# ZeayW/Multimodal-fusion-based-Pre-routing-Timing-Prediction-

Measured on AMD Instinct MI355X. Metric: train-step samples/sec, higher is better.
Workload: dtype bf16; 1 GPU; config B: 8 designs/step/GPU, 65536-node netlist, 64 levels, 256x256 tile, 1350 endpoints/design, UNet(max), bf16 operands / fp32 accumulate on the MFMA-bound contractions; U-Net activations and their gradients stored bf16, netlist tensors, statistics, parameters and gradients fp32; nodes=65536, levels=64, tile=256, endpoints_per_design=1350, cone_pruning=False, parallelism=dp1 (designs sharded, one all-reduce of the flat gradient per step), launch=one HIP graph replay per step (Adam inside)

## Files before the change

multimodal-fusion-based-pre-routing-timing-prediction-_amd/csrc/mlp_feat.hip:

```cpp
#include <stdlib.h>
#include "mlp_tile_bf16.h"
#include "mlp_feat_frag.h"
#include "tr_read.h"
#include "../../include/mmft_incr.h"

namespace mmft {

int launch_slab_reduce(const float* slabs, int splits, long long elems, float* out, int accumulate, hipStream_t st);

struct FeatFwdArgs {
  const float* x;
  long long ldx;
  int row0, n, fin;
  const float *w1, *b1, *w2, *b2;
  float* out;
  long long ldout;
  int relu_out;
  const unsigned char* active;
};

template <int KS, bool MASKED>
__global__ void __launch_bounds__(512) mlp2_feat_fwd_kernel(FeatFwdArgs a) {
  constexpr int BM = 64, RT = BM / 16, XS = KS * 32 + 8, HS = L2_HD + 8;
  __shared__ __attribute__((aligned(16))) unsigned short xs[BM * XS];
  __shared__ __attribute__((aligned(16))) unsigned short hs[BM * HS];
  const int tid = threadIdx.x, lane = tid & 63, wave = tid >> 6;
  const int r16 = lane & 15, q = lane >> 4;
  const int ntiles = (a.n + BM - 1) / BM;
  auto next_tile = [&](int t, unsigned long long& flags) -> int {
    if constexpr (MASKED) {
      for (; t < ntiles; t += (int)gridDim.x) {
        const int m = t * BM + lane;
        flags = __ballot(m < a.n && a.active[a.row0 + m] != 0);
        if (flags) break;
      }
    }
    return t;
  };
  unsigned long long flags = ~0ull;
  int tile = next_tile(blockIdx.x, flags);
  if constexpr (MASKED) {
    if (tile >= ntiles) return;
  }
  bf16x8 w1f[2][KS], w2f[8];
#pragma unroll
  for (int j = 0; j < 2; ++j)
#pragma unroll
    for (int ks = 0; ks < KS; ++ks) w1f[j][ks] = mf_w1_frag(a.w1, a.fin, wave * 32 + j * 16 + r16, ks * 32 + q * 8);
#pragma unroll
  for (int ks = 0; ks < 8; ++ks) w2f[ks] = mf_pack8(a.w2 + (long long)(wave * 16 + r16) * L2_HD + ks * 32 + q * 8);
  const int nn2 = wave * 16 + q * 4;
  const f32x4 b2v = *reinterpret_cast<const f32x4*>(a.b2 + nn2);
  f32x4 b1v[2];
#pragma unroll
  for (int j = 0; j < 2; ++j) b1v[j] = *reinterpret_cast<const f32x4*>(a.b1 + wave * 32 + j * 16 + q * 4);
  constexpr int NXE = BM * KS * 32 / 512;
  float xr[NXE];
  auto request = [&](int tile) {
#pragma unroll
    for (int k = 0; k < NXE; ++k) {
      const int e = tid + k * 512, r = e / (KS * 32), kk = e % (KS * 32);
      const int m = tile * BM + r;
      xr[k] = (m < a.n && kk < a.fin) ? a.x[(long long)(a.row0 + m) * a.ldx + kk] : 0.f;
    }
  };
  if (tile < ntiles) request(tile);
  while (tile < ntiles) {
    const int m0 = tile * BM;
#pragma unroll
    for (int k = 0; k < NXE; ++k) {
      const int e = tid + k * 512;
      xs[(e / (KS * 32)) * XS + e % (KS * 32)] = mf_bf16(xr[k]);
    }
    __syncthreads();
    unsigned long long nflags = ~0ull;
    const int nxt = next_tile(tile + (int)gridDim.x, nflags);
    if (nxt < ntiles) request(nxt);
    f32x4 acc1[RT][2];
    tile_layer1<KS, RT>(acc1, w1f, xs, XS, r16, q);
#pragma unroll
    for (int i = 0; i < RT; ++i)
#pragma unroll
      for (int j = 0; j < 2; ++j) st_bf16x4(hs + (i * 16 + r16) * HS + wave * 32 + j * 16 + q * 4, relu4(acc1[i][j] + b1v[j]));
    __syncthreads();
    f32x4 acc2[RT];
#pragma unroll
    for (int i = 0; i < RT; ++i) acc2[i] = tile_layer2(w2f, hs, HS, r16, q, i);
#pragma unroll
    for (int i = 0; i < RT; ++i) {
      const int m = m0 + i * 16 + r16;
      if (m >= a.n) continue;
      if constexpr (MASKED) {
        if (!((flags >> (i * 16 + r16)) & 1)) continue;
      }
      f32x4 v = acc2[i] + b2v;
      if (a.relu_out) v = relu4(v);
      *reinterpret_cast<f32x4*>(a.out + (long long)(a.row0 + m) * a.ldout + nn2) = v;
    }
    __syncthreads();
    tile = nxt;
    flags = nflags;
  }
}

struct FeatBwdArgs {
  const float* g;
  long long ldg;
  const float* x;
  long long ldx;
  int row0, n, fin;
  const float *w1, *b1, *w2;
  float* slabs;
  long long slab;
};

template <int KS>
__global__ void __launch_bounds__(512) mlp2_feat_bwd_kernel(FeatBwdArgs a) {
  constexpr int BM = 32, KP = KS * 32, XS = KP + 16, GS = L2_D2 + 16, HS = L2_HD + 16, KB = KP / 16;
  extern __shared__ __attribute__((aligned(16))) unsigned short lds[];
  unsigned short* xs = lds;
  unsigned short* gs = xs + BM * XS;
  unsigned short* hs = gs + BM * GS;
  unsigned short* ds = hs + BM * HS;
  f32x4(*gred)[32] = reinterpret_cast<f32x4(*)[32]>(hs);
  const int tid = threadIdx.x, lane = tid & 63, wave = tid >> 6;
  const int r16 = lane & 15, q = lane >> 4;
  const int trr = tr_lane_row(lane), trc = tr_lane_col(lane);
  const f32x4 zero = {0.f, 0.f, 0.f, 0.f};

  bf16x8 w1f[2][KS], w2tf[2][4];
  f32x4 b1v[2];
#pragma unroll
  for (int j = 0; j < 2; ++j) {
    const int col = wave * 32 + j * 16 + r16;
#pragma unroll
    for (int ks = 0; ks < KS; ++ks) w1f[j][ks] = mf_w1_frag(a.w1, a.fin, col, ks * 32 + q * 8);
#pragma unroll
    for (int ks = 0; ks < 4; ++ks) {
      float v[8];
#pragma unroll
      for (int t = 0; t < 8; ++t) v[t] = a.w2[(long long)(ks * 32 + q * 8 + t) * L2_HD + col];
      w2tf[j][ks] = mf_pack8(v);
    }
    b1v[j] = *reinterpret_cast<const f32x4*>(a.b1 + wave * 32 + j * 16 + q * 4);
  }
  f32x4 dw2[2][8], dw1[2][KB], dsum[2], gsum = zero;
#pragma unroll
  for (int j = 0; j < 2; ++j) {
    dsum[j] = zero;
#pragma unroll
    for (int d = 0; d < 8; ++d) dw2[j][d] = zero;
#pragma unroll
    for (int k = 0; k < KB; ++k) dw1[j][k] = zero;
  }

  const int ntiles = (a.n + BM - 1) / BM;
  constexpr int NXE = BM * KP / 512;
  f32x4 gr[2];
  float xr[NXE];
  auto request = [&](int tile) {
    const int m0 = tile * BM;
#pragma unroll
    for (int it = 0; it < 2; ++it) {
      const int e = tid + it * 512, r = e >> 5, c = (e & 31) * 4;
      gr[it] = m0 + r < a.n ? *reinterpret_cast<const f32x4*>(a.g + (long long)(a.row0 + m0 + r) * a.ldg + c) : zero;
    }
#pragma unroll
    for (int k = 0; k < NXE; ++k) {
      const int e = tid + k * 512, r = e / KP, kk = e % KP;
      xr[k] = (m0 + r < a.n && kk < a.fin) ? a.x[(long long)(a.row0 + m0 + r) * a.ldx + kk] : 0.f;
    }
  };
  if ((int)blockIdx.x < ntiles) request(blockIdx.x);
  for (int tile = blockIdx.x; tile < ntiles; tile += gridDim.x) {
#pragma unroll
    for (int it = 0; it < 2; ++it) {
      const int e = tid + it * 512, r = e >> 5, c = (e & 31) * 4;
      const f32x4 v = gr[it];
      gsum += v;
      const unsigned lo = pack_bf16(v.x, v.y), hi = pack_bf16(v.z, v.w);
      *reinterpret_cast<unsigned long long*>(gs + r * GS + c) = ((unsigned long long)hi << 32) | lo;
    }
#pragma unroll
    for (int k = 0; k < NXE; ++k) {
      const int e = tid + k * 512, r = e / KP, kk = e % KP;
      xs[r * XS + kk] = mf_bf16(xr[k]);
    }
    __syncthreads();
    if (tile + (int)gridDim.x < ntiles) request(tile + gridDim.x);
    __syncthreads();
#pragma unroll
    for (int i = 0; i < 2; ++i) {
      f32x4 acc1[2] = {zero, zero}, acc3[2] = {zero, zero};
#pragma unroll
      for (int ks = 0; ks < KS; ++ks) {
        const bf16x8 xf = *reinterpret_cast<const bf16x8*>(xs + (i * 16 + r16) * XS + ks * 32 + q * 8);
#pragma unroll
        for (int j = 0; j < 2; ++j) acc1[j] = __builtin_amdgcn_mfma_f32_16x16x32_bf16(w1f[j][ks], xf, acc1[j], 0, 0, 0);
      }
#pragma unroll
      for (int ks = 0; ks < 4; ++ks) {
        const bf16x8 gf = *reinterpret_cast<const bf16x8*>(gs + (i * 16 + r16) * GS + ks * 32 + q * 8);
#pragma unroll
        for (int j = 0; j < 2; ++j) acc3[j] = __builtin_amdgcn_mfma_f32_16x16x32_bf16(w2tf[j][ks], gf, acc3[j], 0, 0, 0);
      }
      const int m = i * 16 + r16;
#pragma unroll
      for (int j = 0; j < 2; ++j) {
        const int nn = wave * 32 + j * 16 + q * 4;
        f32x4 hv = acc1[j] + b1v[j], dh = acc3[j];
#pragma unroll
        for (int t = 0; t < 4; ++t) {
          hv[t] = hv[t] > 0.f ? hv[t] : 0.f;
          dh[t] = hv[t] > 0.f ? dh[t] : 0.f;
        }
        dsum[j] += dh;
        const unsigned hl = pack_bf16(hv.x, hv.y), hh = pack_bf16(hv.z, hv.w);
        const unsigned dl = pack_bf16(dh.x, dh.y), dhh = pack_bf16(dh.z, dh.w);
        *reinterpret_cast<unsigned long long*>(hs + m * HS + nn) = ((unsigned long long)hh << 32) | hl;
        *reinterpret_cast<unsigned long long*>(ds + m * HS + nn) = ((unsigned long long)dhh << 32) | dl;
      }
    }
    __syncthreads();
#pragma unroll
    for (int j = 0; j < 2; ++j) {
      const int col0 = wave * 32 + j * 16;
      const bf16x8 hf = __builtin_bit_cast(bf16x8, tr_read_pair(hs + trr * HS + col0 + trc, 16 * HS));
      const bf16x8 df = __builtin_bit_cast(bf16x8, tr_read_pair(ds + trr * HS + col0 + trc, 16 * HS));
#pragma unroll
      for (int d = 0; d < 8; ++d) {
        const bf16x8 gf = __builtin_bit_cast(bf16x8, tr_read_pair(gs + trr * GS + d * 16 + trc, 16 * GS));
        dw2[j][d] = __builtin_amdgcn_mfma_f32_16x16x32_bf16(hf, gf, dw2[j][d], 0, 0, 0);
      }
#pragma unroll
      for (int k = 0; k < KB; ++k) {
        const bf16x8 xf = __builtin_bit_cast(bf16x8, tr_read_pair(xs + trr * XS + k * 16 + trc, 16 * XS));
        dw1[j][k] = __builtin_amdgcn_mfma_f32_16x16x32_bf16(df, xf, dw1[j][k], 0, 0, 0);
      }
    }
    __syncthreads();
  }

  float* sl = a.slabs + (long long)blockIdx.x * a.slab;
  float* s_dw1 = sl;
  float* s_db1 = s_dw1 + (long long)L2_HD * a.fin;
  float* s_dw2 = s_db1 + L2_HD;
  float* s_db2 = s_dw2 + (long long)L2_D2 * L2_HD;
#pragma unroll
  for (int j = 0; j < 2; ++j) {
    const int colq = wave * 32 + j * 16 + q * 4;
#pragma unroll
    for (int d = 0; d < 8; ++d) *reinterpret_cast<f32x4*>(s_dw2 + (long long)(d * 16 + r16) * L2_HD + colq) = dw2[j][d];
#pragma unroll
    for (int k = 0; k < KB; ++k) {
      const int kk = k * 16 + r16;
      if (kk < a.fin) {
#pragma unroll
        for (int t = 0; t < 4; ++t) s_dw1[(long long)(colq + t) * a.fin + kk] = dw1[j][k][t];
      }
    }
    f32x4 v = dsum[j];
#pragma unroll
    for (int o = 1; o < 16; o <<= 1) {
#pragma unroll
      for (int t = 0; t < 4; ++t) v[t] += __shfl_xor(v[t], o, 64);
    }
    if (r16 == 0) *reinterpret_cast<f32x4*>(s_db1 + colq) = v;
  }
  __syncthreads();
  gred[tid >> 5][tid & 31] = gsum;
  __syncthreads();
  if (tid < 32) {
    f32x4 v = gred[0][tid];
    for (int p = 1; p < 16; ++p) v += gred[p][tid];
    *reinterpret_cast<f32x4*>(s_db2 + tid * 4) = v;
  }
}

template <int KS>
constexpr int feat_bwd_lds() {
  constexpr int BM = 32, KP = KS * 32, XS = KP + 16, GS = L2_D2 + 16, HS = L2_HD + 16;
  return (BM * XS + BM * GS + 2 * BM * HS) * 2;
}

static inline long long feat_slab(int fin) { return (long long)L2_HD * fin + L2_HD + (long long)L2_D2 * L2_HD + L2_D2; }
static inline int feat_bwd_grid(int n) {
  int tiles = cdiv(n, 32);
  static int cap = getenv("MMFT_FEAT_BWD_GRID") ? atoi(getenv("MMFT_FEAT_BWD_GRID")) : 192;
  if (cap < 1) cap = 1;
  return tiles < cap ? (tiles < 1 ? 1 : tiles) : cap;
}

}

using namespace mmft;

static int feat_fwd_launch(const char* what, const float* x, long long ldx, int row0, int n, int fin, const float* w1,
                           const float* b1, const float* w2, const float* b2, float* out, long long ldout, int relu_out,
                           const unsigned char* active, int device, void* stream) {
  MMFT_REQUIRE(x && w1 && b1 && w2 && b2 && out, "%s: null pointer", what);
  MMFT_REQUIRE(n >= 0 && row0 >= 0 && fin >= 1 && fin <= 64 && ldx >= fin, "%s: bad sizes (fin <= 64)", what);
  MMFT_REQUIRE(ldout % 4 == 0 && aligned16(out) && aligned16(w2) && aligned16(b1) && aligned16(b2),
               "%s: out / w2 / biases must be 16-byte aligned", what);
  if (n == 0) return MMFT_OK;
  DeviceGuard dg(device);
  FeatFwdArgs a{x, ldx, row0, n, fin, w1, b1, w2, b2, out, ldout, relu_out, active};
  const double fl = 2.0 * n * ((double)fin * L2_HD + (double)L2_HD * L2_D2), by = 4.0 * n * ((double)fin + L2_D2);
  int grid = cdiv(n, 64);
  if (grid > 768) grid = 768;
  if (active) {
    if (fin <= 32)
      MMFT_LAUNCH("mlp2_feat_fwd_masked_kernel", fl, by, (mlp2_feat_fwd_kernel<1, true>), dim3(grid), dim3(512), (hipStream_t)stream, a);
    else
      MMFT_LAUNCH("mlp2_feat_fwd_masked_kernel", fl, by, (mlp2_feat_fwd_kernel<2, true>), dim3(grid), dim3(512), (hipStream_t)stream, a);
  } else if (fin <= 32)
    MMFT_LAUNCH("mlp2_feat_fwd_kernel", fl, by, (mlp2_feat_fwd_kernel<1, false>), dim3(grid), dim3(512), (hipStream_t)stream, a);
  else
    MMFT_LAUNCH("mlp2_feat_fwd_kernel", fl, by, (mlp2_feat_fwd_kernel<2, false>), dim3(grid), dim3(512), (hipStream_t)stream, a);
  return check_launch(what);
}

extern "C" int mmft_mlp2_feat_fwd_bf16(const float* x, long long ldx, int row0, int n, int fin, const float* w1, const float* b1,
                                       const float* w2, const float* b2, float* out, long long ldout, int relu_out, int device,
                                       void* stream) {
  return feat_fwd_launch("mlp2_feat_fwd_bf16", x, ldx, row0, n, fin, w1, b1, w2, b2, out, ldout, relu_out, nullptr, device, stream);
}

extern "C" int mmft_mlp2_feat_fwd_bf16_masked(const float* x, long long ldx, int row0, int n, int fin, const float* w1,
                                              const float* b1, const float* w2, const float* b2, float* out, long long ldout,
                                              int relu_out, const unsigned char* active, int device, void* stream) {
  MMFT_REQUIRE(active, "mlp2_feat_fwd_bf16_masked: null pointer (active)");
  return feat_fwd_launch("mlp2_feat_fwd_bf16_masked", x, ldx, row0, n, fin, w1, b1, w2, b2, out, ldout, relu_out, active, device,
                         stream);
}

extern "C" long long mmft_mlp2_feat_bwd_workspace_bytes(int n, int fin) {
  if (n <= 0 || fin < 1 || fin > 64) return 0;
  return (long long)feat_bwd_grid(n) * feat_slab(fin) * 4;
}

extern "C" int mmft_mlp2_feat_bwd_bf16(const float* g, long long ldg, const float* x, long long ldx, int row0, int n, int fin,
                                       const float* w1, const float* b1, const float* w2, float* dw1, float* db1, float* dw2,
                                       float* db2, int accumulate, float* workspace, long long workspace_bytes, int device,
                                       void* stream) {
  MMFT_REQUIRE(g && x && w1 && b1 && w2 && dw1 && db1 && dw2 && db2, "mlp2_feat_bwd_bf16: null pointer");
  MMFT_REQUIRE(n > 0 && row0 >= 0 && fin >= 1 && fin <= 64 && ldx >= fin && ldg >= L2_D2, "mlp2_feat_bwd_bf16: bad sizes (fin <= 64)");
  MMFT_REQUIRE(ldg % 4 == 0 && aligned16(g) && aligned16(b1), "mlp2_feat_bwd_bf16: g / b1 must be 16-byte aligned");
  MMFT_REQUIRE(workspace && aligned16(workspace) && workspace_bytes >= mmft_mlp2_feat_bwd_workspace_bytes(n, fin),
               "mlp2_feat_bwd_bf16: workspace too small");
  DeviceGuard dg(device);
  hipStream_t st = (hipStream_t)stream;
  const int grid = feat_bwd_grid(n);
  const long long slab = feat_slab(fin);
  FeatBwdArgs a{g, ldg, x, ldx, row0, n, fin, w1, b1, w2, workspace, slab};
  const double fl = 2.0 * n * (2.0 * fin * L2_HD + 2.0 * L2_HD * L2_D2), by = 4.0 * n * ((double)fin + L2_D2);
  static DynLdsOnce once[2];
  int arc = fin <= 32 ? ensure_dyn_lds(once[0], reinterpret_cast<const void*>(&mlp2_feat_bwd_kernel<1>), feat_bwd_lds<1>(), "mlp2_feat_bwd_bf16")
                      : ensure_dyn_lds(once[1], reinterpret_cast<const void*>(&mlp2_feat_bwd_kernel<2>), feat_bwd_lds<2>(), "mlp2_feat_bwd_bf16");
  if (arc) return arc;
  if (fin <= 32)
    MMFT_LAUNCH_LDS("mlp2_feat_bwd_kernel", fl, by, mlp2_feat_bwd_kernel<1>, dim3(grid), dim3(512), feat_bwd_lds<1>(), st, a);
  else
    MMFT_LAUNCH_LDS("mlp2_feat_bwd_kernel", fl, by, mlp2_feat_bwd_kernel<2>, dim3(grid), dim3(512), feat_bwd_lds<2>(), st, a);
  int rc = check_launch("mlp2_feat_bwd_bf16");
  if (rc) return rc;
  if (db1 == dw1 + (long long)L2_HD * fin && dw2 == db1 + L2_HD && db2 == dw2 + (long long)L2_D2 * L2_HD && aligned16(dw1))
    return launch_slab_reduce(workspace, grid, slab, dw1, accumulate, st);
  const long long o1 = (long long)L2_HD * fin, o2 = o1 + L2_HD, o3 = o2 + (long long)L2_D2 * L2_HD;
  const SlabSeg segs[4] = {{workspace, dw1, slab, grid, (int)o1, 1, accumulate ? 1 : 0},
                           {workspace + o1, db1, slab, grid, L2_HD, 1, accumulate ? 1 : 0},
                           {workspace + o2, dw2, slab, grid, L2_D2 * L2_HD, 1, accumulate ? 1 : 0},
                           {workspace + o3, db2, slab, grid, L2_D2, 1, accumulate ? 1 : 0}};
  return launch_slab_reduce_batch(segs, 4, st);
}
```

Baseline: 2575 designs/s.

## Tune feature MLP kernels: waves-per-EU hints, W2 in LDS, KB specialization, clamped loads

```diff
diff --git a/multimodal-fusion-based-pre-routing-timing-prediction-_amd/csrc/mlp_feat.hip b/multimodal-fusion-based-pre-routing-timing-prediction-_amd/csrc/mlp_feat.hip
--- a/multimodal-fusion-based-pre-routing-timing-prediction-_amd/csrc/mlp_feat.hip
+++ b/multimodal-fusion-based-pre-routing-timing-prediction-_amd/csrc/mlp_feat.hip
@@ -20,7 +20,8 @@
 };
 
 template <int KS, bool MASKED>
-__global__ void __launch_bounds__(512) mlp2_feat_fwd_kernel(FeatFwdArgs a) {
+__global__ void __launch_bounds__(512) __attribute__((amdgpu_waves_per_eu(MASKED ? 2 : 4, MASKED ? 8 : 4)))
+mlp2_feat_fwd_kernel(FeatFwdArgs a) {
   constexpr int BM = 64, RT = BM / 16, XS = KS * 32 + 8, HS = L2_HD + 8;
   __shared__ __attribute__((aligned(16))) unsigned short xs[BM * XS];
   __shared__ __attribute__((aligned(16))) unsigned short hs[BM * HS];
@@ -114,35 +115,54 @@
   long long slab;
 };
 
+constexpr int FEAT_BWD_WS = L2_D2 + 8;
 template <int KS>
+constexpr bool feat_bwd_w2_lds() { return KS == 2; }
+
+template <int KS, int KB>
 __global__ void __launch_bounds__(512) mlp2_feat_bwd_kernel(FeatBwdArgs a) {
-  constexpr int BM = 32, KP = KS * 32, XS = KP + 16, GS = L2_D2 + 16, HS = L2_HD + 16, KB = KP / 16;
+  constexpr int BM = 32, KP = KS * 32, XS = KP + 16, GS = L2_D2 + 16, HS = L2_HD + 16, WS = FEAT_BWD_WS;
+  static_assert(KB >= 2 * KS - 1 && KB <= 2 * KS, "KB = ceil(fin / 16) with 32 (KS - 1) < fin <= 32 KS");
   extern __shared__ __attribute__((aligned(16))) unsigned short lds[];
   unsigned short* xs = lds;
   unsigned short* gs = xs + BM * XS;
   unsigned short* hs = gs + BM * GS;
   unsigned short* ds = hs + BM * HS;
+  unsigned short* w2s = ds + BM * HS;
   f32x4(*gred)[32] = reinterpret_cast<f32x4(*)[32]>(hs);
   const int tid = threadIdx.x, lane = tid & 63, wave = tid >> 6;
   const int r16 = lane & 15, q = lane >> 4;
   const int trr = tr_lane_row(lane), trc = tr_lane_col(lane);
   const f32x4 zero = {0.f, 0.f, 0.f, 0.f};
 
-  bf16x8 w1f[2][KS], w2tf[2][4];
+  constexpr bool W2LDS = feat_bwd_w2_lds<KS>();
+  bf16x8 w1f[2][KS], w2tf[W2LDS ? 1 : 2][W2LDS ? 1 : 4];
   f32x4 b1v[2];
 #pragma unroll
   for (int j = 0; j < 2; ++j) {
     const int col = wave * 32 + j * 16 + r16;
 #pragma unroll
     for (int ks = 0; ks < KS; ++ks) w1f[j][ks] = mf_w1_frag(a.w1, a.fin, col, ks * 32 + q * 8);
-#pragma unroll
-    for (int ks = 0; ks < 4; ++ks) {
+    if constexpr (!W2LDS) {
+#pragma unroll
+      for (int ks = 0; ks < 4; ++ks) {
+        float v[8];
+#pragma unroll
+        for (int t = 0; t < 8; ++t) v[t] = a.w2[(long long)(ks * 32 + q * 8 + t) * L2_HD + col];
+        w2tf[j][ks] = mf_pack8(v);
+      }
+    }
+    b1v[j] = *reinterpret_cast<const f32x4*>(a.b1 + wave * 32 + j * 16 + q * 4);
+  }
+  if constexpr (W2LDS) {
+#pragma unroll
+    for (int k = 0; k < L2_D2 / 16; ++k) {
+      const int col = tid & (L2_HD - 1), d0 = ((tid >> 8) + 2 * k) * 8;
       float v[8];
 #pragma unroll
-      for (int t = 0; t < 8; ++t) v[t] = a.w2[(long long)(ks * 32 + q * 8 + t) * L2_HD + col];
-      w2tf[j][ks] = mf_pack8(v);
-    }
-    b1v[j] = *reinterpret_cast<const f32x4*>(a.b1 + wave * 32 + j * 16 + q * 4);
+      for (int t = 0; t < 8; ++t) v[t] = a.w2[(d0 + t) * L2_HD + col];
+      *reinterpret_cast<bf16x8*>(w2s + col * WS + d0) = mf_pack8(v);
+    }
   }
   f32x4 dw2[2][8], dw1[2][KB], dsum[2], gsum = zero;
 #pragma unroll
@@ -159,24 +179,29 @@
   f32x4 gr[2];
   float xr[NXE];
   auto request = [&](int tile) {
-    const int m0 = tile * BM;
+    const int m0 = tile * BM, rlast = a.n - 1 - m0, klast = a.fin - 1;
+    const float* gt = a.g + (long long)(a.row0 + m0) * a.ldg;
+    const float* xt = a.x + (long long)(a.row0 + m0) * a.ldx;
+    const unsigned ldg = (unsigned)a.ldg, ldx = (unsigned)a.ldx;
 #pragma unroll
     for (int it = 0; it < 2; ++it) {
       const int e = tid + it * 512, r = e >> 5, c = (e & 31) * 4;
-      gr[it] = m0 + r < a.n ? *reinterpret_cast<const f32x4*>(a.g + (long long)(a.row0 + m0 + r) * a.ldg + c) : zero;
+      gr[it] = *reinterpret_cast<const f32x4*>(gt + ((unsigned)min(r, rlast) * ldg + (unsigned)c));
     }
 #pragma unroll
     for (int k = 0; k < NXE; ++k) {
       const int e = tid + k * 512, r = e / KP, kk = e % KP;
-      xr[k] = (m0 + r < a.n && kk < a.fin) ? a.x[(long long)(a.row0 + m0 + r) * a.ldx + kk] : 0.f;
+      xr[k] = xt[(unsigned)min(r, rlast) * ldx + (unsigned)min(kk, klast)];
     }
   };
   if ((int)blockIdx.x < ntiles) request(blockIdx.x);
+  if constexpr (W2LDS) __syncthreads();
   for (int tile = blockIdx.x; tile < ntiles; tile += gridDim.x) {
+    const int nrow = a.n - tile * BM;
 #pragma unroll
     for (int it = 0; it < 2; ++it) {
       const int e = tid + it * 512, r = e >> 5, c = (e & 31) * 4;
-      const f32x4 v = gr[it];
+      const f32x4 v = r < nrow ? gr[it] : zero;
       gsum += v;
       const unsigned lo = pack_bf16(v.x, v.y), hi = pack_bf16(v.z, v.w);
       *reinterpret_cast<unsigned long long*>(gs + r * GS + c) = ((unsigned long long)hi << 32) | lo;
@@ -184,7 +209,7 @@
 #pragma unroll
     for (int k = 0; k < NXE; ++k) {
       const int e = tid + k * 512, r = e / KP, kk = e % KP;
-      xs[r * XS + kk] = mf_bf16(xr[k]);
+      xs[r * XS + kk] = mf_bf16((r < nrow && kk < a.fin) ? xr[k] : 0.f);
     }
     __syncthreads();
     if (tile + (int)gridDim.x < ntiles) request(tile + gridDim.x);
@@ -202,7 +227,12 @@
       for (int ks = 0; ks < 4; ++ks) {
         const bf16x8 gf = *reinterpret_cast<const bf16x8*>(gs + (i * 16 + r16) * GS + ks * 32 + q * 8);
 #pragma unroll
-        for (int j = 0; j < 2; ++j) acc3[j] = __builtin_amdgcn_mfma_f32_16x16x32_bf16(w2tf[j][ks], gf, acc3[j], 0, 0, 0);
+        for (int j = 0; j < 2; ++j) {
+          bf16x8 wf;
+          if constexpr (W2LDS) wf = *reinterpret_cast<const bf16x8*>(w2s + (wave * 32 + j * 16 + r16) * WS + ks * 32 + q * 8);
+          else wf = w2tf[j][ks];
+          acc3[j] = __builtin_amdgcn_mfma_f32_16x16x32_bf16(wf, gf, acc3[j], 0, 0, 0);
+        }
       }
       const int m = i * 16 + r16;
 #pragma unroll
@@ -280,7 +310,7 @@
 template <int KS>
 constexpr int feat_bwd_lds() {
   constexpr int BM = 32, KP = KS * 32, XS = KP + 16, GS = L2_D2 + 16, HS = L2_HD + 16;
-  return (BM * XS + BM * GS + 2 * BM * HS) * 2;
+  return (BM * XS + BM * GS + 2 * BM * HS + (feat_bwd_w2_lds<KS>() ? L2_HD * FEAT_BWD_WS : 0)) * 2;
 }
 
 static inline long long feat_slab(int fin) { return (long long)L2_HD * fin + L2_HD + (long long)L2_D2 * L2_HD + L2_D2; }
@@ -307,7 +337,9 @@
   FeatFwdArgs a{x, ldx, row0, n, fin, w1, b1, w2, b2, out, ldout, relu_out, active};
   const double fl = 2.0 * n * ((double)fin * L2_HD + (double)L2_HD * L2_D2), by = 4.0 * n * ((double)fin + L2_D2);
   int grid = cdiv(n, 64);
-  if (grid > 768) grid = 768;
+  static int env_cap = getenv("MMFT_FEAT_FWD_GRID") ? atoi(getenv("MMFT_FEAT_FWD_GRID")) : 0;
+  const int cap = env_cap >= 1 ? env_cap : active ? 768 : 512;
+  if (grid > cap) grid = cap;
   if (active) {
     if (fin <= 32)
       MMFT_LAUNCH("mlp2_feat_fwd_masked_kernel", fl, by, (mlp2_feat_fwd_kernel<1, true>), dim3(grid), dim3(512), (hipStream_t)stream, a);
@@ -334,6 +366,15 @@
                          stream);
 }
 
+template <int KS, int KB>
+static int feat_bwd_launch(const FeatBwdArgs& a, int grid, double fl, double by, hipStream_t st) {
+  static DynLdsOnce once;
+  int rc = ensure_dyn_lds(once, reinterpret_cast<const void*>(&mlp2_feat_bwd_kernel<KS, KB>), feat_bwd_lds<KS>(), "mlp2_feat_bwd_bf16");
+  if (rc) return rc;
+  MMFT_LAUNCH_LDS("mlp2_feat_bwd_kernel", fl, by, (mlp2_feat_bwd_kernel<KS, KB>), dim3(grid), dim3(512), feat_bwd_lds<KS>(), st, a);
+  return check_launch("mlp2_feat_bwd_bf16");
+}
+
 extern "C" long long mmft_mlp2_feat_bwd_workspace_bytes(int n, int fin) {
   if (n <= 0 || fin < 1 || fin > 64) return 0;
   return (long long)feat_bwd_grid(n) * feat_slab(fin) * 4;
@@ -346,6 +387,7 @@
   MMFT_REQUIRE(g && x && w1 && b1 && w2 && dw1 && db1 && dw2 && db2, "mlp2_feat_bwd_bf16: null pointer");
   MMFT_REQUIRE(n > 0 && row0 >= 0 && fin >= 1 && fin <= 64 && ldx >= fin && ldg >= L2_D2, "mlp2_feat_bwd_bf16: bad sizes (fin <= 64)");
   MMFT_REQUIRE(ldg % 4 == 0 && aligned16(g) && aligned16(b1), "mlp2_feat_bwd_bf16: g / b1 must be 16-byte aligned");
+  MMFT_REQUIRE(ldx < (1ll << 31) / 32 && ldg < (1ll << 31) / 32, "mlp2_feat_bwd_bf16: 32 rows of x / g must fit 31 bits");
   MMFT_REQUIRE(workspace && aligned16(workspace) && workspace_bytes >= mmft_mlp2_feat_bwd_workspace_bytes(n, fin),
                "mlp2_feat_bwd_bf16: workspace too small");
   DeviceGuard dg(device);
@@ -354,15 +396,10 @@
   const long long slab = feat_slab(fin);
   FeatBwdArgs a{g, ldg, x, ldx, row0, n, fin, w1, b1, w2, workspace, slab};
   const double fl = 2.0 * n * (2.0 * fin * L2_HD + 2.0 * L2_HD * L2_D2), by = 4.0 * n * ((double)fin + L2_D2);
-  static DynLdsOnce once[2];
-  int arc = fin <= 32 ? ensure_dyn_lds(once[0], reinterpret_cast<const void*>(&mlp2_feat_bwd_kernel<1>), feat_bwd_lds<1>(), "mlp2_feat_bwd_bf16")
-                      : ensure_dyn_lds(once[1], reinterpret_cast<const void*>(&mlp2_feat_bwd_kernel<2>), feat_bwd_lds<2>(), "mlp2_feat_bwd_bf16");
-  if (arc) return arc;
-  if (fin <= 32)
-    MMFT_LAUNCH_LDS("mlp2_feat_bwd_kernel", fl, by, mlp2_feat_bwd_kernel<1>, dim3(grid), dim3(512), feat_bwd_lds<1>(), st, a);
-  else
-    MMFT_LAUNCH_LDS("mlp2_feat_bwd_kernel", fl, by, mlp2_feat_bwd_kernel<2>, dim3(grid), dim3(512), feat_bwd_lds<2>(), st, a);
-  int rc = check_launch("mlp2_feat_bwd_bf16");
+  int rc = fin <= 16   ? feat_bwd_launch<1, 1>(a, grid, fl, by, st)
+           : fin <= 32 ? feat_bwd_launch<1, 2>(a, grid, fl, by, st)
+           : fin <= 48 ? feat_bwd_launch<2, 3>(a, grid, fl, by, st)
+                       : feat_bwd_launch<2, 4>(a, grid, fl, by, st);
   if (rc) return rc;
   if (db1 == dw1 + (long long)L2_HD * fin && dw2 == db1 + L2_HD && db2 == dw2 + (long long)L2_D2 * L2_HD && aligned16(dw1))
     return launch_slab_reduce(workspace, grid, slab, dw1, accumulate, st);
```

Result: faster. 2618 designs/s, median of 6 (+1.7%).
